# KieDani/UpliftingTableTennis

Hardware: AMD Instinct MI355X
Metric: frames/sec end-to-end (detect+uplift), 1280x720 (higher is better)
Workload: dtype bf16

## Files before the change

### upliftingtabletennis_amd/csrc/conv.h

```cpp
#pragma once
#include "common.h"
#include "wasb_graph.h"
#include "certify_plan.h"

namespace ttup {

struct PackedConv {
    int cout = 0, cin_total = 0, c0 = 0, k = 1, stride = 1, ck = 32;
    void*  w_dev = nullptr;
    void*  w3_dev = nullptr;
    int    mt3 = 0;
    float* bias_dev = nullptr;
    size_t w_bytes = 0;
};

struct Roi {
    int y0 = 0, y1 = 0, x0 = 0, x1 = 0;
    int sy0 = 0, sy1 = 0, sx0 = 0, sx1 = 0;
    const int* flag = nullptr;
    __host__ __device__ bool outside(int f, int y, int x) const {
        if (f == 2 && sy1 > 0) return y < sy0 || y >= sy1 || x < sx0 || x >= sx1;
        return y < y0 || y >= y1 || x < x0 || x >= x1;
    }
};
// ... 10 lines not shown
    const void* res2 = nullptr;
    const void* res3 = nullptr; int sh3 = 0;
    const int* n_active = nullptr;
    Roi roi;
    const PackedConv* lin16 = nullptr; void* lin16_dst = nullptr;
    const PackedConv* lin32 = nullptr; void* lin32_dst = nullptr;
    const PackedConv* pair = nullptr; void* pair_dst = nullptr; int pair_relu = 0;
};

int pack_conv(const FoldedConv& a, const FoldedConv* b , int cin_pad, int dtype, PackedConv* out);
void free_conv(PackedConv* p);

int launch_conv(const PackedConv& p, const ConvLaunch& l, int dtype, hipStream_t stream);
bool conv_f32_mfma_supported(const PackedConv& p);
int launch_conv_f32_mfma(const PackedConv& p, const ConvLaunch& l, hipStream_t stream);
bool conv_x3_supported(const PackedConv& p);
int launch_conv_x3(const PackedConv& p, const ConvLaunch& l, hipStream_t stream);
int pack_conv_x3(const std::vector<float>& w_tap_cin_cout, int cout, int cin_total, int c0, int k, int stride, PackedConv* out);

int launch_stem(const PackedConv& p1, const PackedConv& p2, const PackedConv& p3, const void* x0, void* t2, void* a1,
                int batch, int h, int w, hipStream_t st, int frames_per_sample = 0);
#define TTUP_LAYOUT_NHWC4_FRAME 2

int launch_bneck_trans(const PackedConv& p1, const PackedConv& p5, const PackedConv& p6, const void* a2, const void* t2,
                       void* b0, void* b1, int batch, int h, int w, hipStream_t st);

struct BBSum {
    const void* terms[3] = {nullptr, nullptr, nullptr}; int shifts[3] = {0, 0, 0}; int n_terms = 0;
    void* ysum = nullptr;
    float* heat = nullptr; const float* head_w = nullptr; float head_bias = 0.f; float* pv = nullptr; long long* pi = nullptr;
};
int bb_chain_tiles_per_img(int h, int w);
int launch_bb_chain(const PackedConv* const* convs, int n_convs, const void* x, void* y, int batch, int h, int w,
                    const PackedConv* follow, void* y_follow, hipStream_t st, const BBSum* sum = nullptr);

int launch_upsum(const void* base, const void* const* terms, const int* shifts, int n_terms, void* dst,
                 int batch, int h, int w, int c, int dtype, hipStream_t stream, const int* n_active = nullptr, const Roi* roi = nullptr);

int launch_nchw_to_nhwc(const float* src, void* dst, int batch, int cin, int cpad, int h, int w, int dtype, hipStream_t stream);
int launch_nhwc_to_nchw(const void* src, float* dst, int batch, int c, int h, int w, int dtype, hipStream_t stream);

int launch_head(const void* src, const float* w_dev, const float* bias_dev, int n_out, float* heat, int batch, int h, int w, int cin,
                int dtype, hipStream_t stream, const int* n_active = nullptr, const Roi* roi = nullptr);

int launch_preprocess(const uint8_t* frames, int n_frames, int src_h, int src_w, int dst_h, int dst_w,
                      void* out, int out_layout, int dtype, int first_triple, int n_triples, int frames_per_sample, hipStream_t stream);

int launch_preprocess_crops(const uint8_t* frames, int n_frames, int src_h, int src_w, int dst_h, int dst_w, float* out,
                            const CropRec* crops_dev, int crop0, const int* n_active_dev, int max_crops, int crop_h, int crop_w,
                            int frames_per_sample, hipStream_t stream);

}
```

### upliftingtabletennis_amd/csrc/conv.hip

```cpp
#include "conv_mfma.h"
#include "conv64.h"
#include "conv_stem.h"
#include "conv_bneck.h"
#include "conv_bb.h"
#include "chain16.h"
#include "conv_pointwise.h"

namespace ttup {

int launch_stem(const PackedConv& p1, const PackedConv& p2, const PackedConv& p3, const void* x0, void* t2, void* a1,
                int batch, int h, int w, hipStream_t st, int frames_per_sample) {
    TTUP_REQUIRE((p1.cout == 64 && p1.cin_total == 16 && p1.k == 3 && p1.stride == 1 && p1.ck == 16) ||
                 (p1.cout == 64 && p1.cin_total == 128 && p1.k == 1 && p1.ck == 32), TTUP_EINVAL, "stem: unexpected conv1 shape");
    TTUP_REQUIRE(p2.cout == 64 && p2.cin_total == 64 && p2.k == 3 && p2.stride == 1 && p2.ck == 32, TTUP_EINVAL, "stem: unexpected conv2 shape");
    TTUP_REQUIRE(p3.cout == 32 && p3.cin_total == 64 && p3.k == 1 && p3.ck == 32, TTUP_EINVAL, "stem: unexpected follower shape");
    StemArgs a;
    a.x0 = (const bf16_t*)x0; a.w1 = (const bf16_t*)p1.w_dev; a.b1 = p1.bias_dev; a.w2 = (const bf16_t*)p2.w_dev; a.b2 = p2.bias_dev;
    a.w3 = (const bf16_t*)p3.w_dev; a.b3 = p3.bias_dev; a.t2 = (bf16_t*)t2; a.a1 = (bf16_t*)a1;
    a.H = h; a.W = w; a.tiles_x = cdiv(w, 32); a.tiles_per_img = a.tiles_x * cdiv(h, 8); a.total_tiles = a.tiles_per_img * batch;
    constexpr size_t SMEM = (size_t)(5 * 4 * 64 * 8 + 2 * 9 * 4 * 64 * 8 + 2 * 340 * 32 + 432 * 16) * 2;
    static_assert(SMEM <= 160 * 1024, "LDS budget");
    TTUP_REQUIRE(frames_per_sample == 0 || frames_per_sample == 1 || frames_per_sample == 3, TTUP_EINVAL, "stem: frames per sample must be 0 (X0 records), 1 or 3");
    const bool k4 = p1.k == 1;
    TTUP_REQUIRE(k4 == (frames_per_sample == 3), TTUP_EINVAL, "stem: the 4-step conv1 packing is the three-frame form");
    const dim3 grid(persistent_grid(a.total_tiles));
    if (k4) return launch_noted(stem_kernel<3, true>, grid, 512, SMEM, st, a, "stem_kernel<3, true>");
    if (frames_per_sample == 1) return launch_noted(stem_kernel<1, false>, grid, 512, SMEM, st, a, "stem_kernel<1, false>");
    return launch_noted(stem_kernel<0, false>, grid, 512, SMEM, st, a, "stem_kernel<0, false>");
}

int launch_bneck_trans(const PackedConv& p1, const PackedConv& p5, const PackedConv& p6, const void* a2, const void* t2,
                       void* b0, void* b1, int batch, int h, int w, hipStream_t st) {
    TTUP_REQUIRE(p1.cout == 128 && p1.cin_total == 96 && p1.c0 == 32 && p1.k == 1 && p1.ck == 32, TTUP_EINVAL, "bneck_trans: unexpected conv1 shape");
    TTUP_REQUIRE(p5.cout == 16 && p5.cin_total == 128 && p5.k == 3 && p5.stride == 1 && p5.ck == 32, TTUP_EINVAL, "bneck_trans: unexpected conv5 shape");
    TTUP_REQUIRE(p6.cout == 32 && p6.cin_total == 128 && p6.k == 3 && p6.stride == 2 && p6.ck == 32, TTUP_EINVAL, "bneck_trans: unexpected conv6 shape");
    TTUP_REQUIRE(h % 2 == 0 && w % 2 == 0, TTUP_EINVAL, "bneck_trans: even input size required");
    FusedArgs a;
    a.a2 = (const bf16_t*)a2; a.t2 = (const bf16_t*)t2;
    a.w1 = (const bf16_t*)p1.w_dev; a.b1 = p1.bias_dev; a.w5 = (const bf16_t*)p5.w_dev; a.b5 = p5.bias_dev;
    a.w6 = (const bf16_t*)p6.w_dev; a.b6 = p6.bias_dev; a.b0 = (bf16_t*)b0; a.b1o = (bf16_t*)b1;
    a.H = h; a.W = w; a.tiles_x = cdiv(w, 32); a.tiles_per_img = a.tiles_x * cdiv(h, 8); a.total_tiles = a.tiles_per_img * batch;
    constexpr size_t SMEM = (size_t)(340 * 128 + 3 * 8 * 64 * 8 + 4 * 9 * 64 * 8) * 2 + 512;
    return launch_noted(bneck_trans_kernel, dim3(persistent_grid(a.total_tiles)), 512, SMEM, st, a, "bneck_trans_kernel");
}

constexpr int BB2_TH = 24, BB2_TW = 32;
int bb_chain_tiles_per_img(int h, int w) { return cdiv(w, BB2_TW) * cdiv(h, BB2_TH); }

int launch_bb_chain(const PackedConv* const* convs, int n_convs, const void* x, void* y, int batch, int h, int w,
                    const PackedConv* follow, void* y_follow, hipStream_t st, const BBSum* sum) {
    TTUP_REQUIRE(n_convs == 2 || n_convs == 4, TTUP_EINVAL, "bb_chain: 2 or 4 convs expected");
    const int c = convs[0]->cout;
    BBArgs a;
    a.x = (const bf16_t*)x; a.y = (bf16_t*)y;
    if (sum) {
        TTUP_REQUIRE(c == 16 && n_convs == 4 && sum->n_terms >= 0 && sum->n_terms <= 3, TTUP_EINVAL, "bb_chain: the fused fuse-layer sum rides on the 16-channel two-block chain");
        TTUP_REQUIRE(sum->ysum || (sum->heat && sum->head_w && sum->pv && sum->pi), TTUP_EINVAL, "bb_chain: fused sum needs an output");
        a.nsum = sum->n_terms; a.ysum = (bf16_t*)sum->ysum;
        for (int k = 0; k < sum->n_terms; ++k) { a.st[k] = (const bf16_t*)sum->terms[k]; a.ssh[k] = sum->shifts[k]; }
        a.heat = sum->heat; a.hw = sum->head_w; a.hbias = sum->head_bias; a.pv = sum->pv; a.pi = sum->pi;
    }
    if (follow) {
        TTUP_REQUIRE(c == 32 && n_convs == 2 && follow->cout == 16 && follow->cin_total == 32 && follow->k == 1 && follow->ck == 32 && y_follow, TTUP_EINVAL,
                     "bb_chain: the fused follower is a 1x1 32->16 conv on a 32-channel block");
        a.wf = (const bf16_t*)follow->w_dev; a.bf = follow->bias_dev; a.yf = (bf16_t*)y_follow;
    }
    for (int i = 0; i < n_convs; ++i) {
        const PackedConv& p = *convs[i];
        TTUP_REQUIRE(p.cout == c && p.cin_total == c && p.k == 3 && p.stride == 1 && p.ck == (c == 16 ? 16 : 32), TTUP_EINVAL, "bb_chain: unexpected conv shape");
        a.w[i] = (const bf16_t*)p.w_dev; a.bias[i] = p.bias_dev;
    }
    if (c == 16 && n_convs == 4) {
        static const bool generic = env_set("TTUP_BB2_GENERIC");
        bool shifts_ok = true;
        for (int k = 0; k < a.nsum && k < 3; ++k) shifts_ok = shifts_ok && a.ssh[k] == k + 1;
        const bool sum_stored = !generic && shifts_ok && a.nsum >= 1 && a.nsum <= 3 && a.ysum && !a.heat;
        const bool tail = !generic && shifts_ok && a.nsum == 3 && a.heat && !a.y && !a.ysum;
        const bool plain = !generic && a.nsum == 0 && !a.heat && !a.ysum && a.y;
        if (plain) return launch_c16_t<BB2_TH, BB2_TW, 4>(a, batch, h, w, st);
        if (tail) return launch_c16_t<BB2_TH, BB2_TW, 7>(a, batch, h, w, st);
        if (sum_stored && a.nsum == 1) return launch_c16_t<BB2_TH, BB2_TW, 1>(a, batch, h, w, st);
        if (sum_stored && a.nsum == 2) return launch_c16_t<BB2_TH, BB2_TW, 2>(a, batch, h, w, st);
        if (sum_stored && a.nsum == 3) return launch_c16_t<BB2_TH, BB2_TW, 3>(a, batch, h, w, st);
        return launch_bb2_t<16, BB2_TH, BB2_TW>(a, batch, h, w, st);
    }
    if (c == 16 && n_convs == 2) return launch_bb_t<16, 8, 32>(a, batch, h, w, st);
    if (c == 32 && n_convs == 2) {
        return launch_bb_t<32, 22, 30>(a, batch, h, w, st);
    }
    set_error("bb_chain: C=%d with %d convs unsupported", c, n_convs);
    return TTUP_EINVAL;
}

void free_conv(PackedConv* p) {
    if (p->w_dev) (void)hipFree(p->w_dev);
    if (p->bias_dev) (void)hipFree(p->bias_dev);
    if (p->w3_dev) (void)hipFree(p->w3_dev);
    p->w_dev = nullptr; p->bias_dev = nullptr; p->w3_dev = nullptr;
}

int pack_conv(const FoldedConv& a, const FoldedConv* b, int cin_pad, int dtype, PackedConv* out) {
    const int k = a.k, taps = k * k, cout = a.cout;
    const int c0 = cin_pad > a.cin ? cin_pad : a.cin;
    const int c1 = b ? b->cin : 0;
    TTUP_REQUIRE(!b || (b->cout == cout && b->k == k && k == 1), TTUP_EINVAL, "two-source conv needs matching 1x1 convs");
    TTUP_REQUIRE(cout % 16 == 0 && cout <= 128, TTUP_EINVAL, "cout %d unsupported", cout);
    const int cin_total = c0 + c1;
    out->cout = cout; out->cin_total = cin_total; out->c0 = c0; out->k = k; out->stride = a.stride;
    std::vector<float> bias(cout);
    for (int i = 0; i < cout; ++i) bias[i] = a.bias[i] + (b ? b->bias[i] : 0.f);
    auto wval = [&](int co, int ci, int tap) -> float {
        if (ci < c0) return ci < a.cin ? a.w[((size_t)co * a.cin + ci) * taps + tap] : 0.f;
        return b->w[((size_t)co * b->cin + (ci - c0)) * taps + tap];
    };
    TTUP_HIP_CHECK(hipMalloc((void**)&out->bias_dev, cout * sizeof(float)));
    TTUP_HIP_CHECK(hipMemcpy(out->bias_dev, bias.data(), cout * sizeof(float), hipMemcpyHostToDevice));
    if (dtype == TTUP_DTYPE_F32) {
        std::vector<float> w((size_t)taps * cin_total * cout);
        for (int t = 0; t < taps; ++t)
            for (int ci = 0; ci < cin_total; ++ci)
                for (int co = 0; co < cout; ++co) w[((size_t)t * cin_total + ci) * cout + co] = wval(co, ci, t);
// ... 168 lines not shown
```

### upliftingtabletennis_amd/csrc/conv_bb.h

```cpp
#pragma once
#include "conv_dev.h"
#include "conv.h"

namespace ttup {

struct BBArgs {
    const bf16_t* x = nullptr; bf16_t* y = nullptr;
    const bf16_t* w[4] = {}; const float* bias[4] = {};
    int H = 0, W = 0, tiles_x = 0, tiles_per_img = 0, total_tiles = 0;
    const bf16_t* wf = nullptr; const float* bf = nullptr; bf16_t* yf = nullptr;
    const bf16_t* st[3] = {}; int ssh[3] = {}; int nsum = 0; bf16_t* ysum = nullptr;
    float* heat = nullptr; const float* hw = nullptr; float hbias = 0.f; float* pv = nullptr; long long* pi = nullptr;
};
struct BBTermLds { const bf16_t* s_terms; int toff[3]; int tw[3]; };

__device__ __forceinline__ float relu_f32(float v) { const int b = __float_as_int(v); return __int_as_float(b > 0 ? b : 0); }
struct BBBest { float v; long long i; };
__device__ __forceinline__ bool bb_better(float v, long long i, float bv, long long bi) {
    const bool vn = v != v, bn = bv != bv;
    if (vn || bn) return vn && (!bn || i < bi);
    return v > bv || (v == bv && i < bi);
}

__device__ __forceinline__ unsigned long long bb_key(float v, int e) {
// ... 16 lines not shown
        case 2: lo = __builtin_amdgcn_update_dpp(0, lo, 0x102, 0xf, 0xf, false); hi = __builtin_amdgcn_update_dpp(0, hi, 0x102, 0xf, 0xf, false); break;
        default: lo = __builtin_amdgcn_update_dpp(0, lo, 0x101, 0xf, 0xf, false); hi = __builtin_amdgcn_update_dpp(0, hi, 0x101, 0xf, 0xf, false); break;
    }
    return ((unsigned long long)hi << 32) | lo;
}

template <int C> __device__ __forceinline__ int bb_off(int pix, int x, int c8) {
    if (C == 32) return pix * 32 + ((c8 ^ ((x >> 1) & 3)) << 3);
    return pix * C + ((c8 ^ ((x >> 2) & 1)) << 3);
}

struct BBFrag16 { bf16x8 af[5]; f32x4 bias; };
__device__ __forceinline__ bf16x8 bb_identity_frag(int lane) {
    const int n = lane & 15, g = lane >> 4;
    unsigned short idm[8];
#pragma unroll
    for (int j = 0; j < 8; ++j) idm[j] = (n == (g & 1) * 8 + j) ? 0x3F80 : 0;
    return __builtin_bit_cast(bf16x8, idm);
}
__device__ __forceinline__ int bb_tap16(int s, int h) {
    return s < 3 ? 3 * s + h : (s == 3 ? (h ? 5 : 2) : (h ? 9 : 8));
}
__device__ __forceinline__ bf16x8 bb_weight_frag16(const bf16_t* wfrag, int s, int lane) {
    const int i = lane & 15, g = lane >> 4, tap = bb_tap16(s, g >> 1);
    return *(const bf16x8*)(wfrag + ((tap >> 1) * 64 + i + 16 * (2 * (tap & 1) + (g & 1))) * 8);
}
__device__ __forceinline__ void bb_load_frag16(BBFrag16& f, const bf16_t* wfrag, const float* biasp, int lane) {
#pragma unroll
    for (int s = 0; s < 5; ++s) f.af[s] = bb_weight_frag16(wfrag, s, lane);
    f.bias = *(const f32x4*)(biasp + (lane >> 4) * 4);
}

template <int R> struct BBRow { static constexpr int value = R; };
template <int C, int RWI, int IOFF, int RHO, int RWO, bool SECOND, int RWR, int ROFF, bool GLOBAL_OUT, int ORW, int OOFF, int NWV = 8>
__device__ __forceinline__ void bb_conv(const bf16_t* s_in, bf16_t* s_out, const bf16_t* s_res, const bf16_t* wfrag, const float* biasp,
                                        bf16_t* gout, int gy0, int gx0, int H, int W, int b, int wave, int lane,
                                        const bf16_t* wf = nullptr, const float* bfp = nullptr, bf16_t* yf = nullptr,
                                        const BBArgs* ex = nullptr, BBBest* best = nullptr, const BBFrag16* pre = nullptr,
                                        const BBTermLds* tl = nullptr, bf16x8 idm_pre = bf16x8{}, const bf16x8* af32 = nullptr) {
    constexpr int MT = C / 16;
    constexpr int KSTEPS = (C == 16) ? 5 : 9;
    constexpr int XT = (RWO + 15) / 16;
    static_assert(NWV == 8 || C == 32, "only the 32-channel row loop takes a wave count");
    const int n = lane & 15, g = lane >> 4;
    bf16x8 af[KSTEPS][MT];
    if (C == 32 && af32) {
#pragma unroll
        for (int s = 0; s < KSTEPS; ++s)
#pragma unroll
            for (int m = 0; m < MT; ++m) af[s][m] = af32[s * MT + m];
    } else if (C == 16 && pre) {
#pragma unroll
        for (int s = 0; s < KSTEPS; ++s) af[s][0] = pre->af[s < 5 ? s : 4];
    } else {
#pragma unroll
        for (int s = 0; s < KSTEPS; ++s)
#pragma unroll
            for (int m = 0; m < MT; ++m) af[s][m] = (C == 16) ? bb_weight_frag16(wfrag, s < 5 ? s : 4, lane) : *(const bf16x8*)(wfrag + ((s * MT + m) * 64 + lane) * 8);
    }
    constexpr bool RES_MFMA = SECOND && C == 16;
    if (RES_MFMA && g >= 2) af[KSTEPS - 1][0] = pre ? idm_pre : bb_identity_frag(lane);
    f32x4 bias[MT];
    if (C == 16 && pre) bias[0] = pre->bias;
    else {
#pragma unroll
        for (int m = 0; m < MT; ++m) bias[m] = *(const f32x4*)(biasp + g * 4 * MT + m * 4);
    }
    int koff[KSTEPS];
#pragma unroll
    for (int s = 0; s < KSTEPS; ++s) {
        const int dy = s / 3, dx = s % 3;
        koff[s] = (dy * RWI + dx) * C + ((g ^ (((n + dx + IOFF) >> 1) & 3)) << 3);
    }
    constexpr int XLAST = (XT - 1) * 16;
    const int nl = (XLAST + n < RWO) ? n : (RWO - 1 - XLAST);
    const int res_ch = (C == 32) ? ((g ^ (((n + ROFF) >> 1) & 3)) << 3) : ((((g >> 1) ^ (((n + ROFF) >> 2) & 1)) << 3) + (g & 1) * 4);
    const int out_ch = (C == 32) ? ((g ^ (((n + OOFF) >> 1) & 3)) << 3) : ((((g >> 1) ^ (((n + OOFF) >> 2) & 1)) << 3) + (g & 1) * 4);
    const bool interior = gy0 >= 0 && gy0 + RHO <= H && gx0 >= 0 && gx0 + RWO <= W;
    constexpr bool CAN_FOLLOW = GLOBAL_OUT && C == 32;
    bf16x8 af_f = {};
    f32x4 bias_f = {0.f, 0.f, 0.f, 0.f};
    if (CAN_FOLLOW && yf) { af_f = *(const bf16x8*)(wf + lane * 8); bias_f = *(const f32x4*)(bfp + g * 4); }
    constexpr bool CAN_SUM = GLOBAL_OUT && C == 16;
    f32x4 hw4 = {0.f, 0.f, 0.f, 0.f};
    if (CAN_SUM && ex && ex->heat) hw4 = *(const f32x4*)(ex->hw + g * 4);
    constexpr bool BAND = (C == 16);
    constexpr int RB = (RHO + 7) / 8;
    const int yb = BAND ? wave * RB : wave;
    const bf16_t* pk0[KSTEPS];
    const bf16_t* pkl[KSTEPS];
    {
        const bf16_t* row0 = s_in + ((wave + IOFF) * RWI + IOFF) * C;
#pragma unroll
        for (int s = 0; s < KSTEPS; ++s) { pk0[s] = row0 + n * C + koff[s]; pkl[s] = row0 + (XLAST + nl) * C + koff[s]; }
    }
    constexpr int ROWSTEP = NWV * RWI * C;
    bf16_t* const so0 = GLOBAL_OUT ? nullptr : s_out + ((yb + OOFF) * ORW + n + OOFF) * C + out_ch;
    const unsigned st_c = (unsigned)((n * C + g * 4 * MT) * 2), st_16 = (unsigned)((n * 16 + g * 4) * 2);
    auto epi = [&](int xt, int orow, int y, const f32x4 (&accx)[MT]) __attribute__((always_inline)) {
        const int gy = gy0 + y;
        const bool row_in = gy >= 0 && gy < H;
        const int x = xt * 16 + n;
        const bool valid = !(xt == XT - 1 && x >= RWO);
        float v[4 * MT];
#pragma unroll
        for (int m = 0; m < MT; ++m)
#pragma unroll
            for (int r = 0; r < 4; ++r) v[m * 4 + r] = accx[m][r];
        if (SECOND && !RES_MFMA) {
            const bf16_t* rp = s_res + ((yb + ROFF) * RWR + n + ROFF) * C + res_ch + (orow * RWR + xt * 16) * C;
            add_bf16x8(v, *(const u32x4*)rp);
        }
        unsigned pk[2 * MT];
#pragma unroll
        for (int i = 0; i < 2 * MT; ++i) pk[i] = relu_pk(pack2(v[2 * i], v[2 * i + 1]));
        const int gx = gx0 + x;
        bool inside = true;
        if (!interior) {
            inside = row_in && gx >= 0 && gx < W;
#pragma unroll
            for (int i = 0; i < 2 * MT; ++i) pk[i] = inside ? pk[i] : 0u;
// ... 30 lines not shown
                                       bf16_to_f32((bf16_t)(q1 & 0xffff)), bf16_to_f32((bf16_t)(q1 >> 16))};
                        if (exact_tail) {
#pragma unroll
                            for (int r = 0; r < 4; ++r) hy[r] = ys[r] > 0.f ? ys[r] : 0.f;
                        }
                        float part = hy[0] * hw4[0];
                        part = fmaf(hy[1], hw4[1], part);
                        part = fmaf(hy[2], hw4[2], part);
                        part = fmaf(hy[3], hw4[3], part);
                        part += __shfl_xor(part, 16, 64);
                        part += __shfl_xor(part, 32, 64);
                        const float hv = part + ex->hbias;
                        if (live && g == 0) {
                            const long long e = (long long)gy * W + gx;
                            ex->heat[(size_t)b * H * W + e] = hv;
                            if (bb_better(hv, e, best->v, best->i)) { best->v = hv; best->i = e; }
                        }
                    }
                }
            }
            if constexpr (CAN_FOLLOW) {
                if (yf) {
                    const u32x4 bq = u32x4{pk[0], pk[1], pk[2], pk[3]};
                    const f32x4 cf = __builtin_amdgcn_mfma_f32_16x16x32_bf16(af_f, __builtin_bit_cast(bf16x8, bq), bias_f, 0, 0, 0);
                    if (inside && valid) *(u32x2*)((char*)(yf + rowpix * 16) + (opaque_u32(st_16) + (unsigned)(xt * 16 * 32))) = u32x2{pack2(cf[0], cf[1]), pack2(cf[2], cf[3])};
                }
            }
        } else if (valid) {
            bf16_t* o = so0 + (orow * ORW + xt * 16) * C;
            if (C == 16) *(u32x2*)o = u32x2{pk[0], pk[1]};
            else *(u32x4*)o = u32x4{pk[0], pk[1], pk[2], pk[3]};
        }
    };
    if constexpr (!BAND) {
        constexpr int ROW_UNROLL = (RHO + NWV - 1) / NWV;
#pragma unroll ROW_UNROLL
        for (int yj = 0; yj < (RHO + NWV - 1) / NWV; ++yj) {
            const int y = wave + NWV * yj;
            if (y >= RHO) break;
            f32x4 acc[XT][MT];
#pragma unroll
            for (int xt = 0; xt < XT; ++xt)
#pragma unroll
                for (int m = 0; m < MT; ++m) acc[xt][m] = bias[m];
            bf16x8 bfr[2][XT];
            auto load_step = [&](int s, bf16x8 (&bf)[XT]) __attribute__((always_inline)) {
#pragma unroll
                for (int xt = 0; xt < XT; ++xt)
                    bf[xt] = (xt < XT - 1) ? *(const bf16x8*)(pk0[s] + yj * ROWSTEP + xt * 16 * C) : *(const bf16x8*)(pkl[s] + yj * ROWSTEP);
            };
            load_step(0, bfr[0]);
#pragma unroll
            for (int s = 0; s < KSTEPS; ++s) {
                if (s + 1 < KSTEPS) load_step(s + 1, bfr[(s + 1) & 1]);
                __builtin_amdgcn_sched_barrier(0);
#pragma unroll
                for (int xt = 0; xt < XT; ++xt)
#pragma unroll
                    for (int m = 0; m < MT; ++m) acc[xt][m] = __builtin_amdgcn_mfma_f32_16x16x32_bf16(af[s][m], bfr[s & 1][xt], acc[xt][m], 0, 0, 0);
                __builtin_amdgcn_sched_barrier(0);
            }
#pragma unroll
            for (int xt = 0; xt < XT; ++xt) epi(xt, NWV * yj, y, acc[xt]);
        }
    } else {
        const int h = g >> 1, c8 = g & 1;
        constexpr int RS = RWI * C;
// ... 73 lines not shown
                    valid = p < NSP;
                    const int pc = valid ? p : NSP - 1;
                    row = pc / RX; col = XLAST + (pc - row * RX);
                }
                const bf16_t* b0 = s_in + ((row + IOFF) * RWI + IOFF + col) * C;
                const int sw2 = (c8 ^ (((col + 2 + IOFF) >> 2) & 1)) << 3;
                const bf16_t* a0 = b0 + h * C + ((c8 ^ (((col + h + IOFF) >> 2) & 1)) << 3);
                const bf16_t* a3 = b0 + h * RS + 2 * C + sw2;
                const bf16_t* a4 = b0 + 2 * RS + 2 * C + sw2;
                if (RES_MFMA && h) a4 = s_res + ((row + ROFF) * RWR + ROFF + col) * C + ((c8 ^ (((col + ROFF) >> 2) & 1)) << 3);
                f32x4 acc = __builtin_amdgcn_mfma_f32_16x16x32_bf16(af[0][0], *(const bf16x8*)a0, bias[0], 0, 0, 0);
                acc = __builtin_amdgcn_mfma_f32_16x16x32_bf16(af[1][0], *(const bf16x8*)(a0 + RS), acc, 0, 0, 0);
                acc = __builtin_amdgcn_mfma_f32_16x16x32_bf16(af[2][0], *(const bf16x8*)(a0 + 2 * RS), acc, 0, 0, 0);
                acc = __builtin_amdgcn_mfma_f32_16x16x32_bf16(af[3][0], *(const bf16x8*)a3, acc, 0, 0, 0);
                acc = __builtin_amdgcn_mfma_f32_16x16x32_bf16(af[4][0], *(const bf16x8*)a4, acc, 0, 0, 0);
                unsigned q0 = relu_pk(pack2(acc[0], acc[1])), q1 = relu_pk(pack2(acc[2], acc[3]));
                if (!interior) {
                    const int gy = gy0 + row, gx = gx0 + col;
                    const bool inside = gy >= 0 && gy < H && gx >= 0 && gx < W;
                    q0 = inside ? q0 : 0u; q1 = inside ? q1 : 0u;
                }
                if (valid) *(u32x2*)(s_out + ((row + OOFF) * ORW + col + OOFF) * C + ((((g >> 1) ^ (((col + OOFF) >> 2) & 1)) << 3) + (g & 1) * 4)) = u32x2{q0, q1};
            };
            if (wave == 7) {
#pragma unroll
                for (int j = 0; j < K0; ++j) strip(j);
            }
            if (K0 + wave < NSG) strip(K0 + wave);
            if (NSG - K0 > 8 && K0 + 8 + wave < NSG) strip(K0 + 8 + wave);
        }
    }
}

template <int C, int NB, int TH, int TW>
__global__ __launch_bounds__(512) void bb_chain_kernel(BBArgs a) {
    static_assert(NB == 1, "one BasicBlock; the two-block chain is bb_chain2_kernel / c16_chain_kernel");
    constexpr int L = 2;
    constexpr int R0H = TH + 2 * L, R0W = TW + 2 * L;
    constexpr int SZ_A = R0H * R0W * C, SZ_B = (R0H - 2) * (R0W - 2) * C;
    constexpr int KSTEPS = (C == 16) ? 5 : 9, MT = C / 16;
    constexpr int W_UNITS = KSTEPS * MT * 64;
    constexpr bool RESIDENT = (C == 32);
    constexpr int W_PT = (W_UNITS + 511) / 512;
    constexpr int IN_UNITS = R0H * R0W * (C / 8), IN_PT = (IN_UNITS + 511) / 512;
    extern __shared__ __attribute__((aligned(16))) char smem[];
    bf16_t* bufA = (bf16_t*)smem;
    bf16_t* bufB = bufA + SZ_A;
    bf16_t* s_wt = bufB + SZ_B;
    float* s_misc = (float*)(s_wt + (RESIDENT ? 2 * W_UNITS * 8 : 0));
    const int tid = threadIdx.x, lane = tid & 63, wave = __builtin_amdgcn_readfirstlane(tid >> 6);
    const int my_tiles = (a.total_tiles - (int)blockIdx.x + (int)gridDim.x - 1) / (int)gridDim.x;

    u32x4 pin[IN_PT];
    unsigned voff[IN_PT];
#pragma unroll
    for (int k = 0; k < IN_PT; ++k) {
        const int u = tid + k * 512;
        const int c8 = u % (C / 8), pix = u / (C / 8);
        voff[k] = u < IN_UNITS ? (unsigned)((((pix / R0W) * a.W + pix % R0W) * C + c8 * 8) * 2) : 0u;
    }
    auto issue_in = [&](int it) {
        const TileAt t = tile_at<TH, TW, L>(xcd_tile(blockIdx.x + it * gridDim.x, a.total_tiles), a.tiles_per_img, a.tiles_x);
        const int b = t.b, gy0 = t.y0, gx0 = t.x0;
        if (gy0 >= 0 && gy0 + R0H <= a.H && gx0 >= 0 && gx0 + R0W <= a.W) {
            const char* base = (const char*)(a.x + ((size_t)(b * a.H + gy0) * a.W + gx0) * C);
#pragma unroll
            for (int k = 0; k < IN_PT; ++k) pin[k] = *(const u32x4*)(base + opaque_u32(voff[k]));
            return;
        }
#pragma unroll
        for (int k = 0; k < IN_PT; ++k) {
            const int u = tid + k * 512;
            const int c8 = u % (C / 8), pix = u / (C / 8);
            const int gy = gy0 + pix / R0W, gx = gx0 + pix % R0W;
            pin[k] = u32x4{0u, 0u, 0u, 0u};
            if (u < IN_UNITS && gy >= 0 && gy < a.H && gx >= 0 && gx < a.W) pin[k] = *(const u32x4*)(a.x + ((size_t)(b * a.H + gy) * a.W + gx) * C + c8 * 8);
        }
    };
// ... 6 lines not shown
            for (int k = 0; k < W_PT; ++k) { const int u = tid + k * 512; pw2[cv][k] = u32x4{0u, 0u, 0u, 0u}; if (u < W_UNITS) pw2[cv][k] = ((const u32x4*)a.w[cv])[u]; }
#pragma unroll
        for (int cv = 0; cv < 2; ++cv)
#pragma unroll
            for (int k = 0; k < W_PT; ++k) { const int u = tid + k * 512; if (u < W_UNITS) ((u32x4*)(s_wt + cv * W_UNITS * 8))[u] = pw2[cv][k]; }
        if (tid < C) { s_misc[tid] = a.bias[0][tid]; s_misc[C + tid] = a.bias[1][tid]; }
        if (a.yf) {
            if (tid < 16) s_misc[2 * C + tid] = a.bf[tid];
            if (tid >= 64 && tid < 128) ((u32x4*)(s_misc + 2 * C + 16))[tid - 64] = ((const u32x4*)a.wf)[tid - 64];
        }
    } else {
        if (my_tiles > 0) issue_in(0);
    }

    if (my_tiles <= 0) return;
    if (RESIDENT) prefetch_arrived(pin);
    for (int it = 0; it < my_tiles; ++it) {
        const TileAt tile = tile_at<TH, TW>(xcd_tile(blockIdx.x + it * gridDim.x, a.total_tiles), a.tiles_per_img, a.tiles_x);
        const int b = tile.b, oy0 = tile.y0, ox0 = tile.x0;
        __syncthreads();
#pragma unroll
        for (int k = 0; k < IN_PT; ++k) {
            const int u = tid + k * 512;
            if (u < IN_UNITS) { const int c8 = u % (C / 8), pix = u / (C / 8); *(u32x4*)(bufA + bb_off<C>(pix, pix % R0W, c8)) = pin[k]; }
        }
        __syncthreads();
        if (it + 1 < my_tiles) issue_in(it + 1);
        const bf16_t* w0 = RESIDENT ? s_wt : a.w[0];
        const bf16_t* w1 = RESIDENT ? s_wt + W_UNITS * 8 : a.w[1];
        const float* bias0 = RESIDENT ? s_misc : a.bias[0];
        const float* bias1 = RESIDENT ? s_misc + C : a.bias[1];
        const bf16_t* wfl = RESIDENT ? (const bf16_t*)(s_misc + 2 * C + 16) : a.wf;
        const float* bfl = RESIDENT ? s_misc + 2 * C : a.bf;
        bb_conv<C, R0W, 0, R0H - 2, R0W - 2, false, 1, 0, false, R0W - 2, 0>(bufA, bufB, nullptr, w0, bias0, nullptr, oy0 - 1, ox0 - 1, a.H, a.W, b, wave, lane);
        __syncthreads();
        if (RESIDENT) prefetch_arrived(pin);
        bb_conv<C, R0W - 2, 0, TH, TW, true, R0W, 2, true, 1, 0>(bufB, nullptr, bufA, w1, bias1, a.y, oy0, ox0, a.H, a.W, b, wave, lane, wfl, bfl, a.yf);
    }
}

template <int C, int TH, int TW>
__global__ __launch_bounds__(512, 4) void bb_chain2_kernel(BBArgs a) {
    constexpr int L = 4;
    constexpr int R0H = TH + 2 * L, R0W = TW + 2 * L;
    constexpr int SA = (R0W & 1) ? R0W : R0W + 1;
    constexpr int SB = ((R0W - 2) & 1) ? R0W - 2 : R0W - 1;
    constexpr int SZ_A = R0H * SA * C;
    constexpr int SZ_B = (R0H - 2) * SB * C;
    extern __shared__ __attribute__((aligned(16))) char smem[];
    bf16_t* bufA = (bf16_t*)smem;
    bf16_t* bufB = bufA + SZ_A;
    const int tid = threadIdx.x, lane = tid & 63, wave = __builtin_amdgcn_readfirstlane(tid >> 6);
    const int bx = (gridDim.x & 7) == 0 ? (blockIdx.x & 7) * (gridDim.x >> 3) + (blockIdx.x >> 3) : blockIdx.x;
    const int b = blockIdx.z, tt = blockIdx.y * a.tiles_x + bx;
    const int oy0 = blockIdx.y * TH, ox0 = bx * TW;
    BBFrag16 fr;
    {
        constexpr int CU = R0W * (C / 8);
        constexpr int RL = 512 / CU;
        constexpr int IN_PT = (R0H + RL - 1) / RL;
        static_assert(RL >= 1, "tile row wider than the workgroup");
        const int cu = tid % CU, rl = tid / CU;
        const int col = cu / (C / 8), c8 = cu % (C / 8);
        const int gx = ox0 - L + col, gyb = oy0 - L + rl;
        const bool col_ok = rl < RL && gx >= 0 && gx < a.W;
        const bf16_t* src = a.x + ((long long)(b * a.H + gyb) * a.W + gx) * C + c8 * 8;
        const long long row_step = (long long)RL * a.W * C;
        u32x4 v[IN_PT];
#pragma unroll
        for (int k = 0; k < IN_PT; ++k) {
            const int gy = gyb + k * RL;
// ... 59 lines not shown
            if (bb_better(ov, oi, best.v, best.i)) { best.v = ov; best.i = oi; }
        }
        __syncthreads();
        float* sv = (float*)smem; long long* si = (long long*)(smem + 64);
        if (lane == 0) { sv[wave] = best.v; si[wave] = best.i; }
        __syncthreads();
        if (tid == 0) {
            for (int k = 1; k < 8; ++k) if (bb_better(sv[k], si[k], best.v, best.i)) { best.v = sv[k]; best.i = si[k]; }
            a.pv[(size_t)b * a.tiles_per_img + tt] = best.v;
            a.pi[(size_t)b * a.tiles_per_img + tt] = best.i;
        }
    }
}

template <int TH, int TW>
static BBArgs bb_tiled(const BBArgs& a, int batch, int h, int w) {
    BBArgs k = a;
    k.H = h; k.W = w; k.tiles_x = cdiv(w, TW); k.tiles_per_img = k.tiles_x * cdiv(h, TH); k.total_tiles = k.tiles_per_img * batch;
    return k;
}

template <int C, int TH, int TW>
static int launch_bb2_t(const BBArgs& a, int batch, int h, int w, hipStream_t st) {
    constexpr int SA = ((TW + 8) & 1) ? TW + 8 : TW + 9, SB = ((TW + 6) & 1) ? TW + 6 : TW + 7;
    constexpr size_t SMEM = (size_t)((TH + 8) * SA + (TH + 6) * SB) * C * 2 + 64;
    static_assert(SMEM <= 160 * 1024, "LDS budget");
    static_assert(2 * SMEM <= 160 * 1024 || TH * TW > 24 * 32, "the 24x32 tile runs two workgroups per CU");
    const BBArgs k = bb_tiled<TH, TW>(a, batch, h, w);
    return launch_noted(bb_chain2_kernel<C, TH, TW>, dim3(k.tiles_x, cdiv(h, TH), batch), 512, SMEM, st, k, "bb_chain2_kernel<%d, %d, %d>", C, TH, TW);
}

constexpr int BB_MISC_BYTES = (2 * 32 + 16) * 4 + 1024;
template <int C, int TH, int TW>
static int launch_bb_t(const BBArgs& a, int batch, int h, int w, hipStream_t st) {
    constexpr int KSTEPS = (C == 16) ? 5 : 9, MT = C / 16;
    constexpr size_t SMEM = (size_t)((TH + 4) * (TW + 4) + (TH + 2) * (TW + 2)) * C * 2 +
                            (C == 16 ? 0 : (size_t)2 * KSTEPS * MT * 1024 + BB_MISC_BYTES);
    static_assert(SMEM <= 160 * 1024, "LDS budget");
    const BBArgs k = bb_tiled<TH, TW>(a, batch, h, w);
    const int per_cu = (int)((160 * 1024) / SMEM) > 2 ? 2 : ((int)((160 * 1024) / SMEM) < 1 ? 1 : (int)((160 * 1024) / SMEM));
    const int grid = C == 16 ? k.total_tiles : persistent_grid(k.total_tiles, per_cu);
    return launch_noted(bb_chain_kernel<C, 1, TH, TW>, dim3(grid), 512, SMEM, st, k, "bb_chain_kernel<%d, 1, %d, %d>", C, TH, TW);
}

}
```

### upliftingtabletennis_amd/csrc/wasb_net.h

```cpp
#pragma once
#include "conv.h"

namespace ttup {
size_t upsum_head_ws_bytes(int n_maps, int H, int W);
int launch_upsum_head(const void* base, const void* const* terms, const int* shifts, int n_terms, const float* w_dev, float bias,
                      float* heat, int n_maps, int H, int W, long long* argmax, float* win, void* ws, size_t ws_bytes, hipStream_t st);
int refine_argmax(const float* heat, int n_maps, int H, int W, long long* argmax, float* win, void* ws, size_t ws_bytes, hipStream_t st);
int launch_argmax_finish(const float* heat, int n_maps, int H, int W, int nblk, const float* pv, const long long* pi, long long* argmax, float* win, hipStream_t st);

struct Tensor : TensorShape { void* ptr = nullptr; };

struct CertState {
    bool enabled = false;
    float eps = 0.f;
    static constexpr float GUARD = 1.25f;
    int R = CERT_R;
    int small = 0;
    int K = 256;
    int maxc = 8;
    int maxf = 8;
    int CH = 0, nchunks = 0, max_crops = 0, Hc = 0, Wc = 0;
    int budget = 0;
    bool exact_windows = false;
    int audit_mod = 0, audit_phase = 0;
// ... 4 lines not shown
        int* guard_cnt = nullptr;
        int* status = nullptr; int* n_crops = nullptr;
        int* cand_idx = nullptr; int* cand_crop = nullptr; float* cand_val = nullptr; float* cand_win = nullptr;
        float* cand_bf = nullptr;
        CropRec* crop_rec = nullptr; int* n_active = nullptr;
        int* roi_flag = nullptr;
        float* margin = nullptr;
        hipEvent_t done = nullptr;
        hipEvent_t read_status = nullptr, read_info = nullptr, read_margin = nullptr;
    } slot[2];
    int cur = 0;
    unsigned long long* stats = nullptr;
    float* crop_heat = nullptr;
    hipStream_t stream = nullptr;
    hipEvent_t lanes_done = nullptr;
};
}

struct ttup_wasb {
    int H = 0, W = 0, max_batch = 0, dtype = 0, micro = 1, in_ch = 9;
    std::vector<ttup::PackedConv> convs;
    std::vector<ttup::Tensor> tensors;
    std::vector<ttup::Op> ops;
    std::map<std::string, int> taps;
    int t_input = -1, t_out = -1;
    int t_frames = -1;
    bool frames_mode = false;
    float* head_w_dev = nullptr; float* head_b_dev = nullptr; float head_bias = 0.f;
    int n_out = 1;
    float* heat_scratch = nullptr;
    void* refine_ws = nullptr; size_t refine_ws_bytes = 0;
    long long* argmax_scratch = nullptr; float* win_scratch = nullptr;
    int last_batch = 0;
    bool fused_head = false;
    const int* n_active = nullptr;
    std::vector<ttup::Roi> op_roi; ttup::Roi out_roi; const int* roi_flag = nullptr;
    std::vector<char> blob;
    ttup::CertState cert;
    struct Lane {
        std::vector<void*> ptr;
        float* heat_scratch = nullptr; void* refine_ws = nullptr; long long* argmax_scratch = nullptr; float* win_scratch = nullptr;
        hipStream_t stream = nullptr; hipEvent_t done = nullptr;
    };
    std::vector<Lane> lanes;
    hipEvent_t fork = nullptr;
    hipEvent_t pass_done = nullptr;
    bool pass_recorded = false;

    void use_lane(int l) {
        const Lane& L = lanes[l];
        for (size_t i = 0; i < tensors.size(); ++i) tensors[i].ptr = L.ptr[i];
        heat_scratch = L.heat_scratch; refine_ws = L.refine_ws; argmax_scratch = L.argmax_scratch; win_scratch = L.win_scratch;
    }
    size_t esize() const { return dtype == TTUP_DTYPE_F32 ? 4 : 2; }
    ~ttup_wasb();
};

namespace ttup {
int run_ops(ttup_wasb* net, int mb, hipStream_t st);
int compute_roi(ttup_wasb* net, int lo, int hi, int lo2 = 0, int hi2 = 0);
void cert_free(ttup_wasb* net);
int cert_begin(ttup_wasb* net, int batch, hipStream_t caller);
int cert_scan(ttup_wasb* net, const float* heat, const long long* argmax, int b0, int mb, hipStream_t st);
int cert_finish(ttup_wasb* net, const float* x_dev, const uint8_t* frames_dev, int n_frames, int src_h, int src_w, int batch,
                int64_t* argmax_dev, float* win_dev, hipStream_t caller);
}
// ... 1 lines not shown
```

### upliftingtabletennis_amd/csrc/wasb_net.hip

```cpp
#include "wasb_net.h"
#include "wasb_blob.h"
#include <string.h>
#include <stdlib.h>
#include <memory>

using namespace ttup;

ttup_wasb::~ttup_wasb() {
    cert_free(this);
    for (auto& c : convs) free_conv(&c);
    for (auto& L : lanes) {
        for (void* q : L.ptr) if (q) (void)hipFree(q);
        if (L.heat_scratch) (void)hipFree(L.heat_scratch);
        if (L.refine_ws) (void)hipFree(L.refine_ws);
        if (L.argmax_scratch) (void)hipFree(L.argmax_scratch);
        if (L.win_scratch) (void)hipFree(L.win_scratch);
        if (L.stream) (void)hipStreamDestroy(L.stream);
        if (L.done) (void)hipEventDestroy(L.done);
    }
    if (fork) (void)hipEventDestroy(fork);
    if (pass_done) (void)hipEventDestroy(pass_done);
    if (head_w_dev) (void)hipFree(head_w_dev);
    if (head_b_dev) (void)hipFree(head_b_dev);
}
// ... 11 lines not shown
        const Tensor& s = net->tensors[op.src0];
        ConvLaunch l;
        l.src0 = s.ptr; l.src1 = op.src1 >= 0 ? net->tensors[op.src1].ptr : nullptr;
        l.residual = op.residual >= 0 ? net->tensors[op.residual].ptr : nullptr;
        l.dst = net->tensors[op.dst].ptr; l.batch = mb; l.h = s.h; l.w = s.w; l.relu = op.relu; l.n_active = net->n_active;
        if (!net->op_roi.empty() && net->roi_flag) { l.roi = net->op_roi[&op - net->ops.data()]; l.roi.flag = net->roi_flag; }
        if (op.conv2 >= 0) { l.follow = &net->convs[op.conv2]; l.dst2 = net->tensors[op.dst2].ptr; }
        if (op.lin16 >= 0) { l.lin16 = &net->convs[op.lin16]; l.lin16_dst = net->tensors[op.lin16_dst].ptr; }
        if (op.lin32 >= 0) { l.lin32 = &net->convs[op.lin32]; l.lin32_dst = net->tensors[op.lin32_dst].ptr; }
        if (op.pair >= 0) { l.pair = &net->convs[op.pair]; l.pair_dst = net->tensors[op.pair_dst].ptr; l.pair_relu = op.pair_relu; }
        if (op.res2 >= 0) l.res2 = net->tensors[op.res2].ptr;
        if (op.res3 >= 0) { l.res3 = net->tensors[op.res3].ptr; l.sh3 = op.sh3; }
        const int rc = launch_conv(net->convs[op.conv], l, net->dtype, st);
        if (rc) return rc;
    } else if (op.kind == Op::STEM) {
        const Tensor& s = net->tensors[op.src0];
        const bool fm = net->frames_mode && net->t_frames >= 0 && op.conv1f >= 0;
        const int rc = launch_stem(net->convs[fm ? op.conv1f : op.conv], net->convs[op.conv2], net->convs[op.conv3], fm ? net->tensors[net->t_frames].ptr : s.ptr,
                                   net->tensors[op.dst].ptr, net->tensors[op.dst2].ptr, mb, s.h, s.w, st, fm ? net->in_ch / 3 : 0);
        if (rc) return rc;
    } else if (op.kind == Op::UPSUM_HEAD) {
        return TTUP_OK;
    } else if (op.kind == Op::BB_CHAIN) {
        if (op.head) return TTUP_OK;
        const Tensor& s = net->tensors[op.src0];
        const PackedConv* cv[4]; BBSum sum;
        chain_args(net, op, cv, &sum);
        int rc;
        if (op.n_chain == 4 && op.n_terms > 0) {
            sum.ysum = net->tensors[op.dst2].ptr;
            rc = launch_bb_chain(cv, 4, s.ptr, op.dst >= 0 ? net->tensors[op.dst].ptr : nullptr, mb, s.h, s.w, nullptr, nullptr, st, &sum);
        } else {
            rc = launch_bb_chain(cv, op.n_chain, s.ptr, net->tensors[op.dst].ptr, mb, s.h, s.w,
                                 op.conv2 >= 0 ? &net->convs[op.conv2] : nullptr, op.dst2 >= 0 ? net->tensors[op.dst2].ptr : nullptr, st);
        }
        if (rc) return rc;
    } else if (op.kind == Op::BNECK_TRANS) {
        const Tensor& s = net->tensors[op.src0];
        const int rc = launch_bneck_trans(net->convs[op.conv], net->convs[op.conv2], net->convs[op.conv3], s.ptr, net->tensors[op.src1].ptr,
                                          net->tensors[op.dst].ptr, net->tensors[op.dst2].ptr, mb, s.h, s.w, st);
        if (rc) return rc;
    } else {
        const Tensor& d = net->tensors[op.dst];
        const void* terms[3] = {nullptr, nullptr, nullptr};
        for (int k = 0; k < op.n_terms; ++k) terms[k] = net->tensors[op.terms[k]].ptr;
        Roi roi;
        if (!net->op_roi.empty() && net->roi_flag) { roi = net->op_roi[&op - net->ops.data()]; roi.flag = net->roi_flag; }
        const int rc = launch_upsum(net->tensors[op.src0].ptr, terms, op.shifts, op.n_terms, d.ptr, mb, d.h, d.w, d.c, net->dtype, st, net->n_active, &roi);
        if (rc) return rc;
    }
    return TTUP_OK;
}

int run_graph(ttup_wasb* net, int mb, hipStream_t st) {
    for (const Op& op : net->ops) { const int rc = run_op(net, op, mb, st); if (rc) return rc; }
    return TTUP_OK;
}

int run_head_op(ttup_wasb* net, int mb, float* heat, long long* am, float* wn, hipStream_t st) {
    const Op& op = net->ops.back();
    if (op.kind == Op::BB_CHAIN) {
        const Tensor& s = net->tensors[op.src0];
        const int nblk = bb_chain_tiles_per_img(s.h, s.w);
        TTUP_REQUIRE(net->refine_ws && net->refine_ws_bytes >= (size_t)mb * nblk * 12, TTUP_EINVAL, "head: workspace too small");
        const PackedConv* cv[4]; BBSum sum;
        chain_args(net, op, cv, &sum);
        sum.heat = heat; sum.head_w = net->head_w_dev; sum.head_bias = net->head_bias;
// ... 151 lines not shown
    }
    net->out_roi = Roi();
    net->out_roi.y0 = lo; net->out_roi.y1 = hi; net->out_roi.x0 = lo; net->out_roi.x1 = hi;
    if (two) { net->out_roi.sy0 = lo2; net->out_roi.sy1 = hi2; net->out_roi.sx0 = lo2; net->out_roi.sx1 = hi2; }
    return TTUP_OK;
}
}

int ttup_wasb_create_internal(const void* blob, size_t blob_bytes, int height, int width, int max_batch, int dtype, int micro_override, int lanes_override, ttup_wasb** out) {
    TTUP_REQUIRE(blob && out, TTUP_EINVAL, "ttup_wasb_create: null pointer");
    TTUP_REQUIRE(height > 0 && width > 0 && height % 8 == 0 && width % 8 == 0, TTUP_EINVAL,
                 "ttup_wasb_create: input size %dx%d must be positive multiples of 8", height, width);
    TTUP_REQUIRE(max_batch > 0, TTUP_EINVAL, "ttup_wasb_create: max_batch must be positive");
    TTUP_REQUIRE(dtype == TTUP_DTYPE_BF16 || dtype == TTUP_DTYPE_F32, TTUP_EINVAL, "ttup_wasb_create: unknown dtype %d", dtype);
    std::vector<FoldedConv> folded;
    std::vector<float> head_w, head_b;
    int in_ch = 0, head_out = 0;
    int rc = parse_blob(blob, blob_bytes, &folded, &in_ch, &head_out, &head_w, &head_b);
    if (rc) return rc;
    TTUP_REQUIRE((in_ch == 9 || in_ch == 3) && head_out >= 1 && head_out <= 16, TTUP_EFORMAT, "wasb blob: in_ch=%d head_out=%d unsupported (ball detector 9/3, table detector 3/13)", in_ch, head_out);
    int ndev = 0;
    TTUP_HIP_CHECK(hipGetDeviceCount(&ndev));
    TTUP_REQUIRE(ndev > 0, TTUP_EHIP, "ttup_wasb_create: no HIP device");
    std::unique_ptr<ttup_wasb> net(new ttup_wasb);
    net->H = height; net->W = width; net->max_batch = max_batch; net->dtype = dtype; net->in_ch = in_ch;
    net->blob.assign((const char*)blob, (const char*)blob + blob_bytes);
    net->n_out = head_out == 3 ? 1 : head_out;
    int micro = micro_override > 0 ? micro_override : (int)env_ll("TTUP_MICRO_BATCH", 8);
    if (micro < 1) micro = 1;
    net->micro = micro < max_batch ? micro : max_batch;
    GraphSwitches sw;
    sw.fuse = !env_set("TTUP_NO_FUSE"); sw.fuse_sum = !env_set("TTUP_NO_FUSE_SUM"); sw.fuse_lin = !env_set("TTUP_NO_FUSE_LIN");
    sw.pair = !env_set("TTUP_NO_PAIR"); sw.stem = !env_set("TTUP_NO_STEM"); sw.frames_mode = !env_set("TTUP_NO_FRAMES_MODE");
    const GraphPlan plan = build_graph(folded, in_ch, net->n_out, height, width, net->micro, dtype, sw);
    if (plan.rc) return plan.rc;
    net->ops = plan.ops; net->taps = plan.taps;
    net->t_input = plan.t_input; net->t_out = plan.t_out; net->t_frames = plan.t_frames; net->fused_head = plan.fused_head;
    for (const TensorShape& s : plan.tensors) { Tensor t; static_cast<TensorShape&>(t) = s; net->tensors.push_back(t); }
    for (const ConvRequest& r : plan.convs) {
        net->convs.emplace_back();
        PackedConv& p = net->convs.back();
        rc = pack_conv(plan.source_a(r, folded), r.b >= 0 ? &folded[r.b] : nullptr, r.cin_pad, dtype, &p);
        if (rc) return rc;
        TTUP_REQUIRE(p.cout == r.cout && p.cin_total == r.cin_total && p.c0 == r.c0 && p.k == r.k && p.stride == r.stride, TTUP_EINVAL,
                     "wasb: conv %zu was packed as %d x %d+%d, k %d / s%d; the plan has %d x %d+%d, k %d / s%d", net->convs.size() - 1,
                     p.cout, p.c0, p.cin_total - p.c0, p.k, p.stride, r.cout, r.c0, r.cin_total - r.c0, r.k, r.stride);
    }
    {
        const int first = head_out == 3 ? 1 : 0;
        TTUP_HIP_CHECK(hipMalloc((void**)&net->head_w_dev, (size_t)net->n_out * 16 * sizeof(float)));
        TTUP_HIP_CHECK(hipMemcpy(net->head_w_dev, head_w.data() + (size_t)first * 16, (size_t)net->n_out * 16 * sizeof(float), hipMemcpyHostToDevice));
        TTUP_HIP_CHECK(hipMalloc((void**)&net->head_b_dev, (size_t)net->n_out * sizeof(float)));
        TTUP_HIP_CHECK(hipMemcpy(net->head_b_dev, head_b.data() + first, (size_t)net->n_out * sizeof(float), hipMemcpyHostToDevice));
        net->head_bias = head_b[first];
    }
    const size_t hw = (size_t)height * width;
    net->refine_ws_bytes = ttup_refine_workspace_bytes(net->micro * net->n_out, height, width);
    if (upsum_head_ws_bytes(net->micro, height, width) > net->refine_ws_bytes) net->refine_ws_bytes = upsum_head_ws_bytes(net->micro, height, width);
    {
        int n_lanes = lanes_override > 0 ? lanes_override : (int)env_ll("TTUP_LANES", 2);
        const int n_micro = (max_batch + net->micro - 1) / net->micro;
        if (n_lanes > n_micro) n_lanes = n_micro;
        if (n_lanes < 1) n_lanes = 1;
        if (n_lanes > 4) n_lanes = 4;
        net->lanes.resize(n_lanes);
        for (int l = 0; l < n_lanes; ++l) {
// ... 117 lines not shown
```

Before: 2243.

## Split 32-channel BasicBlock convs into per-wave row bands with rolling accumulators

Adds a banded row schedule for the 32-channel BasicBlock conv. Each wave owns a contiguous band of rows (3/3/3 or 3/3/2 splits) instead of strided rows, and keeps three rolling accumulators so each loaded input row fragment is reused across the three vertical taps. This is meant to cut LDS reads per MFMA. The banded form becomes the default, and the old row-strided kernel stays available behind TTUP_BB32_ROWS. The cost is more live accumulator registers and an uneven rows-per-wave split.

```diff
diff --git a/upliftingtabletennis_amd/csrc/conv.h b/upliftingtabletennis_amd/csrc/conv.h
--- a/upliftingtabletennis_amd/csrc/conv.h
+++ b/upliftingtabletennis_amd/csrc/conv.h
@@ -66,7 +66,7 @@
 };
 int bb_chain_tiles_per_img(int h, int w);
 int launch_bb_chain(const PackedConv* const* convs, int n_convs, const void* x, void* y, int batch, int h, int w,
-                    const PackedConv* follow, void* y_follow, hipStream_t st, const BBSum* sum = nullptr);
+                    const PackedConv* follow, void* y_follow, hipStream_t st, const BBSum* sum = nullptr, bool bb32_rows = false);
 
 int launch_upsum(const void* base, const void* const* terms, const int* shifts, int n_terms, void* dst,
                  int batch, int h, int w, int c, int dtype, hipStream_t stream, const int* n_active = nullptr, const Roi* roi = nullptr);
diff --git a/upliftingtabletennis_amd/csrc/conv.hip b/upliftingtabletennis_amd/csrc/conv.hip
--- a/upliftingtabletennis_amd/csrc/conv.hip
+++ b/upliftingtabletennis_amd/csrc/conv.hip
@@ -48,7 +48,7 @@
 int bb_chain_tiles_per_img(int h, int w) { return cdiv(w, BB2_TW) * cdiv(h, BB2_TH); }
 
 int launch_bb_chain(const PackedConv* const* convs, int n_convs, const void* x, void* y, int batch, int h, int w,
-                    const PackedConv* follow, void* y_follow, hipStream_t st, const BBSum* sum) {
+                    const PackedConv* follow, void* y_follow, hipStream_t st, const BBSum* sum, bool bb32_rows) {
     TTUP_REQUIRE(n_convs == 2 || n_convs == 4, TTUP_EINVAL, "bb_chain: 2 or 4 convs expected");
     const int c = convs[0]->cout;
     BBArgs a;
@@ -86,7 +86,7 @@
     }
     if (c == 16 && n_convs == 2) return launch_bb_t<16, 8, 32>(a, batch, h, w, st);
     if (c == 32 && n_convs == 2) {
-        return launch_bb_t<32, 22, 30>(a, batch, h, w, st);
+        return launch_bb_t<32, 22, 30>(a, batch, h, w, st, bb32_rows);
     }
     set_error("bb_chain: C=%d with %d convs unsupported", c, n_convs);
     return TTUP_EINVAL;
diff --git a/upliftingtabletennis_amd/csrc/conv_bb.h b/upliftingtabletennis_amd/csrc/conv_bb.h
--- a/upliftingtabletennis_amd/csrc/conv_bb.h
+++ b/upliftingtabletennis_amd/csrc/conv_bb.h
@@ -72,7 +72,8 @@
 }
 
 template <int R> struct BBRow { static constexpr int value = R; };
-template <int C, int RWI, int IOFF, int RHO, int RWO, bool SECOND, int RWR, int ROFF, bool GLOBAL_OUT, int ORW, int OOFF, int NWV = 8>
+template <int C, int RWI, int IOFF, int RHO, int RWO, bool SECOND, int RWR, int ROFF, bool GLOBAL_OUT, int ORW, int OOFF, int NWV = 8,
+          bool BAND32 = false, int RA = 0, int RY1 = 0, int RY2 = 0>
 __device__ __forceinline__ void bb_conv(const bf16_t* s_in, bf16_t* s_out, const bf16_t* s_res, const bf16_t* wfrag, const float* biasp,
                                         bf16_t* gout, int gy0, int gx0, int H, int W, int b, int wave, int lane,
                                         const bf16_t* wf = nullptr, const float* bfp = nullptr, bf16_t* yf = nullptr,
@@ -82,6 +83,7 @@
     constexpr int KSTEPS = (C == 16) ? 5 : 9;
     constexpr int XT = (RWO + 15) / 16;
     static_assert(NWV == 8 || C == 32, "only the 32-channel row loop takes a wave count");
+    static_assert(!BAND32 || (C == 32 && NWV == 8 && 4 * RA + 2 * RY1 + 2 * RY2 == RHO), "the band split covers the 32-channel conv's rows");
     const int n = lane & 15, g = lane >> 4;
     bf16x8 af[KSTEPS][MT];
     if (C == 32 && af32) {
@@ -126,7 +128,8 @@
     if (CAN_SUM && ex && ex->heat) hw4 = *(const f32x4*)(ex->hw + g * 4);
     constexpr bool BAND = (C == 16);
     constexpr int RB = (RHO + 7) / 8;
-    const int yb = BAND ? wave * RB : wave;
+    const int yb = BAND32 ? (wave < 4 ? wave * RA : (wave < 6 ? 4 * RA + (wave - 4) * RY1 : 4 * RA + 2 * RY1 + (wave - 6) * RY2))
+                          : (BAND ? wave * RB : wave);
     const bf16_t* pk0[KSTEPS];
     const bf16_t* pkl[KSTEPS];
     {
@@ -223,7 +226,54 @@
             else *(u32x4*)o = u32x4{pk[0], pk[1], pk[2], pk[3]};
         }
     };
-    if constexpr (!BAND) {
+    if constexpr (BAND32) {
+        constexpr int RBM = RA > RY1 ? (RA > RY2 ? RA : RY2) : (RY1 > RY2 ? RY1 : RY2);
+        constexpr int RS = RWI * C;
+        const int rows = wave < 4 ? RA : (wave < 6 ? RY1 : RY2);
+        const bf16_t* row0 = s_in + ((yb + IOFF) * RWI + IOFF) * C;
+        const bf16_t* pb[3];
+        const bf16_t* pbl[3];
+#pragma unroll
+        for (int dx = 0; dx < 3; ++dx) {
+            pb[dx] = row0 + n * C + koff[dx];
+            pbl[dx] = row0 + (XLAST + nl) * C + koff[dx];
+        }
+        auto load_frag = [&](int i, int dx, bf16x8 (&f)[XT]) __attribute__((always_inline)) {
+#pragma unroll
+            for (int xt = 0; xt < XT; ++xt) f[xt] = (xt < XT - 1) ? *(const bf16x8*)(pb[dx] + i * RS + xt * 16 * C) : *(const bf16x8*)(pbl[dx] + i * RS);
+        };
+        if (rows > 0) {
+            f32x4 acc[3][XT][MT];
+            bf16x8 fr[3][XT];
+#pragma unroll
+            for (int dx = 0; dx < 3; ++dx) load_frag(0, dx, fr[dx]);
+#pragma unroll
+            for (int i = 0; i < RBM + 2; ++i) {
+                if (i >= rows + 2) break;
+#pragma unroll
+                for (int dx = 0; dx < 3; ++dx) {
+                    __builtin_amdgcn_sched_barrier(0);
+#pragma unroll
+                    for (int dy = 2; dy >= 0; --dy) {
+                        const int j = i - dy;
+                        if (j < 0 || j >= RBM) continue;
+                        if (j >= rows) continue;
+#pragma unroll
+                        for (int xt = 0; xt < XT; ++xt)
+#pragma unroll
+                            for (int m = 0; m < MT; ++m)
+                                acc[j % 3][xt][m] = __builtin_amdgcn_mfma_f32_16x16x32_bf16(af[dy * 3 + dx][m], fr[dx][xt], (dy == 0 && dx == 0) ? bias[m] : acc[j % 3][xt][m], 0, 0, 0);
+                    }
+                    __builtin_amdgcn_sched_barrier(0);
+                    if (i + 1 < RBM + 2 && i + 1 < rows + 2) load_frag(i + 1, dx, fr[dx]);
+                }
+                if (i >= 2) {
+#pragma unroll
+                    for (int xt = 0; xt < XT; ++xt) epi(xt, i - 2, yb + i - 2, acc[(i - 2) % 3][xt]);
+                }
+            }
+        }
+    } else if constexpr (!BAND) {
         constexpr int ROW_UNROLL = (RHO + NWV - 1) / NWV;
 #pragma unroll ROW_UNROLL
         for (int yj = 0; yj < (RHO + NWV - 1) / NWV; ++yj) {
@@ -363,9 +413,10 @@
     }
 }
 
-template <int C, int NB, int TH, int TW>
-__global__ __launch_bounds__(512) void bb_chain_kernel(BBArgs a) {
-    static_assert(NB == 1, "one BasicBlock; the two-block chain is bb_chain2_kernel / c16_chain_kernel");
+#define BB32_SPLIT1 3, 3, 3
+#define BB32_SPLIT2 3, 3, 2
+template <int C, int TH, int TW, bool BANDS>
+__device__ __forceinline__ void bb_chain_tiles(const BBArgs& a, char* smem) {
     constexpr int L = 2;
     constexpr int R0H = TH + 2 * L, R0W = TW + 2 * L;
     constexpr int SZ_A = R0H * R0W * C, SZ_B = (R0H - 2) * (R0W - 2) * C;
@@ -374,7 +425,6 @@
     constexpr bool RESIDENT = (C == 32);
     constexpr int W_PT = (W_UNITS + 511) / 512;
     constexpr int IN_UNITS = R0H * R0W * (C / 8), IN_PT = (IN_UNITS + 511) / 512;
-    extern __shared__ __attribute__((aligned(16))) char smem[];
     bf16_t* bufA = (bf16_t*)smem;
     bf16_t* bufB = bufA + SZ_A;
     bf16_t* s_wt = bufB + SZ_B;
@@ -447,11 +497,26 @@
         const float* bias1 = RESIDENT ? s_misc + C : a.bias[1];
         const bf16_t* wfl = RESIDENT ? (const bf16_t*)(s_misc + 2 * C + 16) : a.wf;
         const float* bfl = RESIDENT ? s_misc + 2 * C : a.bf;
-        bb_conv<C, R0W, 0, R0H - 2, R0W - 2, false, 1, 0, false, R0W - 2, 0>(bufA, bufB, nullptr, w0, bias0, nullptr, oy0 - 1, ox0 - 1, a.H, a.W, b, wave, lane);
+        if constexpr (BANDS) bb_conv<C, R0W, 0, R0H - 2, R0W - 2, false, 1, 0, false, R0W - 2, 0, 8, true, BB32_SPLIT1>(bufA, bufB, nullptr, w0, bias0, nullptr, oy0 - 1, ox0 - 1, a.H, a.W, b, wave, lane);
+        else bb_conv<C, R0W, 0, R0H - 2, R0W - 2, false, 1, 0, false, R0W - 2, 0>(bufA, bufB, nullptr, w0, bias0, nullptr, oy0 - 1, ox0 - 1, a.H, a.W, b, wave, lane);
         __syncthreads();
         if (RESIDENT) prefetch_arrived(pin);
-        bb_conv<C, R0W - 2, 0, TH, TW, true, R0W, 2, true, 1, 0>(bufB, nullptr, bufA, w1, bias1, a.y, oy0, ox0, a.H, a.W, b, wave, lane, wfl, bfl, a.yf);
-    }
+        if constexpr (BANDS) bb_conv<C, R0W - 2, 0, TH, TW, true, R0W, 2, true, 1, 0, 8, true, BB32_SPLIT2>(bufB, nullptr, bufA, w1, bias1, a.y, oy0, ox0, a.H, a.W, b, wave, lane, wfl, bfl, a.yf);
+        else bb_conv<C, R0W - 2, 0, TH, TW, true, R0W, 2, true, 1, 0>(bufB, nullptr, bufA, w1, bias1, a.y, oy0, ox0, a.H, a.W, b, wave, lane, wfl, bfl, a.yf);
+    }
+}
+
+template <int C, int NB, int TH, int TW>
+__global__ __launch_bounds__(512) void bb_chain_kernel(BBArgs a) {
+    static_assert(NB == 1, "one BasicBlock; the two-block chain is bb_chain2_kernel / c16_chain_kernel");
+    extern __shared__ __attribute__((aligned(16))) char smem[];
+    bb_chain_tiles<C, TH, TW, C == 32>(a, smem);
+}
+template <int C, int NB, int TH, int TW>
+__global__ __launch_bounds__(512) void bb_chain_rows_kernel(BBArgs a) {
+    static_assert(C == 32 && NB == 1, "the row-strided form of the 32-channel block");
+    extern __shared__ __attribute__((aligned(16))) char smem[];
+    bb_chain_tiles<C, TH, TW, false>(a, smem);
 }
 
 template <int C, int TH, int TW>
@@ -577,7 +642,7 @@
 
 constexpr int BB_MISC_BYTES = (2 * 32 + 16) * 4 + 1024;
 template <int C, int TH, int TW>
-static int launch_bb_t(const BBArgs& a, int batch, int h, int w, hipStream_t st) {
+static int launch_bb_t(const BBArgs& a, int batch, int h, int w, hipStream_t st, bool rows32 = false) {
     constexpr int KSTEPS = (C == 16) ? 5 : 9, MT = C / 16;
     constexpr size_t SMEM = (size_t)((TH + 4) * (TW + 4) + (TH + 2) * (TW + 2)) * C * 2 +
                             (C == 16 ? 0 : (size_t)2 * KSTEPS * MT * 1024 + BB_MISC_BYTES);
@@ -585,6 +650,9 @@
     const BBArgs k = bb_tiled<TH, TW>(a, batch, h, w);
     const int per_cu = (int)((160 * 1024) / SMEM) > 2 ? 2 : ((int)((160 * 1024) / SMEM) < 1 ? 1 : (int)((160 * 1024) / SMEM));
     const int grid = C == 16 ? k.total_tiles : persistent_grid(k.total_tiles, per_cu);
+    if constexpr (C == 32) {
+        if (rows32) return launch_noted(bb_chain_rows_kernel<C, 1, TH, TW>, dim3(grid), 512, SMEM, st, k, "bb_chain_rows_kernel<%d, 1, %d, %d>", C, TH, TW);
+    }
     return launch_noted(bb_chain_kernel<C, 1, TH, TW>, dim3(grid), 512, SMEM, st, k, "bb_chain_kernel<%d, 1, %d, %d>", C, TH, TW);
 }
 
diff --git a/upliftingtabletennis_amd/csrc/wasb_net.h b/upliftingtabletennis_amd/csrc/wasb_net.h
--- a/upliftingtabletennis_amd/csrc/wasb_net.h
+++ b/upliftingtabletennis_amd/csrc/wasb_net.h
@@ -60,6 +60,7 @@
     void* refine_ws = nullptr; size_t refine_ws_bytes = 0;
     long long* argmax_scratch = nullptr; float* win_scratch = nullptr;
     int last_batch = 0;
+    bool bb32_rows = false;
     bool fused_head = false;
     const int* n_active = nullptr;
     std::vector<ttup::Roi> op_roi; ttup::Roi out_roi; const int* roi_flag = nullptr;
diff --git a/upliftingtabletennis_amd/csrc/wasb_net.hip b/upliftingtabletennis_amd/csrc/wasb_net.hip
--- a/upliftingtabletennis_amd/csrc/wasb_net.hip
+++ b/upliftingtabletennis_amd/csrc/wasb_net.hip
@@ -67,7 +67,7 @@
             rc = launch_bb_chain(cv, 4, s.ptr, op.dst >= 0 ? net->tensors[op.dst].ptr : nullptr, mb, s.h, s.w, nullptr, nullptr, st, &sum);
         } else {
             rc = launch_bb_chain(cv, op.n_chain, s.ptr, net->tensors[op.dst].ptr, mb, s.h, s.w,
-                                 op.conv2 >= 0 ? &net->convs[op.conv2] : nullptr, op.dst2 >= 0 ? net->tensors[op.dst2].ptr : nullptr, st);
+                                 op.conv2 >= 0 ? &net->convs[op.conv2] : nullptr, op.dst2 >= 0 ? net->tensors[op.dst2].ptr : nullptr, st, nullptr, net->bb32_rows);
         }
         if (rc) return rc;
     } else if (op.kind == Op::BNECK_TRANS) {
@@ -285,6 +285,7 @@
     GraphSwitches sw;
     sw.fuse = !env_set("TTUP_NO_FUSE"); sw.fuse_sum = !env_set("TTUP_NO_FUSE_SUM"); sw.fuse_lin = !env_set("TTUP_NO_FUSE_LIN");
     sw.pair = !env_set("TTUP_NO_PAIR"); sw.stem = !env_set("TTUP_NO_STEM"); sw.frames_mode = !env_set("TTUP_NO_FRAMES_MODE");
+    net->bb32_rows = env_set("TTUP_BB32_ROWS");
     const GraphPlan plan = build_graph(folded, in_ch, net->n_out, height, width, net->micro, dtype, sw);
     if (plan.rc) return plan.rc;
     net->ops = plan.ops; net->taps = plan.taps;
```

Result: no change. 2251, median of 6 (+0.4%).
